# sundy-li/strawboat

Measured on AMD Instinct MI355X. Metric: encode+decode GB/s (uncompressed Arrow bytes) per GPU; 1/2/4/8-GPU scaling, higher is better.
Workload: dtype f64 bit patterns (integer/bit work, no arithmetic); 1 GPU; C2: 512 x 1M-row nullable Float64 columns per GPU, 64Ki-row pages, codec adaptive, inputs resident in HBM; columns_per_gpu=512, rows_per_column=1000000, page_rows=65536, parallelism=pages of independent columns sharded across 1 GPU(s)

## Files before the change

### strawboat_amd/csrc/sb_encode.hip

```cpp
#include <cstring>
#include <type_traits>
#include <utility>
#include <vector>

#include "sb_host.h"
#include "sb_lz4.h"
#include "sb_zstd_enc.h"

namespace sb {

struct EncCol {
    const uint8_t* values;
    const uint8_t* validity;
    const uint8_t* offsets;
    const uint8_t* heads;
    uint8_t* out;
    uint64_t values_bit_offset;
    uint64_t values_len;
    uint64_t values_len_total;
    uint64_t validity_bit_offset;
    uint64_t out_cap;
    uint64_t rows;
    int32_t ptype;
    int32_t nullable;
// ... 3056 lines not shown
#include "sb_select_big.h"
#include "sb_dict_big.h"
#include "sb_bin_page.h"

constexpr uint32_t BIN_LDS_SLOTS = 16384;

constexpr uint32_t BH_ROWS = 2048;
#ifndef BV_ROWS_
#define BV_ROWS_ 4096
#endif
constexpr uint32_t BV_ROWS = BV_ROWS_;
__global__ void __launch_bounds__(WG) k_enc_bin_hash(EncodeArgs a) {
    const uint32_t page = blockIdx.x + a.page_base;
    const EncPage p = get_page(a, page);
    if (p.codec != CODEC_ON_DEVICE || p.h64_off == ~0ull) return;
    const uint64_t r0 = (uint64_t)blockIdx.y * BH_ROWS;
    if (r0 >= p.rows) return;
    if (bp_page_done(a, p, page)) return;
    const EncCol c = get_col(a, p.col);
    const uint64_t r1 = min(p.rows, r0 + BH_ROWS);
    uint64_t* h64 = (uint64_t*)(a.scratch + p.h64_off);
    auto body = [&](auto bk) {
        constexpr int U = 8;
        for (uint64_t base = r0 + threadIdx.x; base < r1; base += (uint64_t)WG * U) {
            uint64_t b[U], e[U];
#pragma unroll
            for (int u = 0; u < U; u++) {
                const uint64_t i = base + (uint64_t)u * WG;
                const uint64_t ic = i < r1 ? i : r0;
                b[u] = bk.beg(ic);
                e[u] = bk.beg(ic + 1);
            }
#pragma unroll
            for (int u = 0; u < U; u++) {
                const uint64_t i = base + (uint64_t)u * WG;
                if (i < r1) gst64(h64 + i, bin_hash_bytes(bk.values, b[u], e[u], c.values_len));
            }
        }
    };
    const ValidView vv{c.validity, c.validity_bit_offset + p.row0};
    if (c.ptype == SB_TYPE_BINARY)
        body(BinKeys<int32_t>{c.offsets + p.row0 * 4, c.values, vv});
    else if (c.ptype == SB_TYPE_LARGE_BINARY)
        body(BinKeys<int64_t>{c.offsets + p.row0 * 8, c.values, vv});
}

__global__ void __launch_bounds__(WG) k_enc_bin_verify(EncodeArgs a, uint32_t tiles_per_page) {
    const uint32_t lin = blockIdx.x, xcd = lin & 7, j = lin >> 3;
    const uint32_t pidx = (j / tiles_per_page) * 8 + xcd, tile = j % tiles_per_page;
    if (pidx >= a.n_pages) return;
    const uint32_t page = pidx + a.page_base;
    const EncPage p = get_page(a, page);
    if (p.codec != CODEC_ON_DEVICE || p.h64_off == ~0ull || !p.aux_bytes) return;
    const uint64_t r0 = (uint64_t)tile * BV_ROWS;
    if (r0 >= p.rows) return;
    if (bp_page_done(a, p, page)) return;
    uint32_t* aux = (uint32_t*)(a.scratch + p.aux_off);
    if (!bh_fits(p.rows, p.aux_bytes)) return;
    const uint32_t magic = gld32(aux + BH_W_MAGIC);
    if (magic != BH_MAGIC && magic != BH_TAGS_USED) return;
    if (a.flags & SB_WRITE_DEBUG_VERIFY_FAIL_BIT) {
        if (threadIdx.x == 0 && tile == 0) atomicOr(aux + BH_W_BAD, 1u);
        return;
    }
    const EncCol c = get_col(a, p.col);
    const uint64_t r1 = min(p.rows, r0 + BV_ROWS);
    const ValidView vv{c.validity, c.validity_bit_offset + p.row0};
    const uint16_t* slot16 = (const uint16_t*)(aux + BH_W_SLOT16);
    const uint16_t* rep16 = (const uint16_t*)(aux + BH_W_REP16);
    const uint64_t* h64 = (const uint64_t*)(a.scratch + p.h64_off);
    bool ok = true;
    auto body = [&](auto keys) {
        using KT = decltype(keys);
        constexpr int VU = 8;
        constexpr bool O32 = sizeof(keys.k.beg(0)) == 8 && std::is_same<KT, BinKeysHashed<int32_t>>::value;
        const uint8_t* offs = keys.k.offs;
        const uint8_t* values = keys.k.values;
        const uint64_t vlen = c.values_len;
        for (uint64_t base = r0 + threadIdx.x; base < r1; base += (uint64_t)WG * VU) {
            uint32_t g[VU];
            uint64_t br[VU], er[VU], bg[VU], eg[VU];
            bool need[VU];
#pragma unroll
            for (int u = 0; u < VU; u++) {
                const uint64_t row = base + (uint64_t)u * WG;
                const uint64_t rc = row < r1 ? row : r0;
                g[u] = ldu16((const uint8_t*)(rep16 + ldu16((const uint8_t*)(slot16 + rc))));
                need[u] = row < r1 && g[u] != (uint32_t)rc;
                if (!need[u]) g[u] = (uint32_t)rc;
            }
#pragma unroll
            for (int u = 0; u < VU; u++) {
                const uint64_t row = base + (uint64_t)u * WG;
                const uint64_t rc = row < r1 ? row : r0;
                if constexpr (O32) {
                    const uint64_t pr = ldu64(offs + rc * 4), pg = ldu64(offs + (uint64_t)g[u] * 4);
                    br[u] = (uint32_t)pr; er[u] = pr >> 32; bg[u] = (uint32_t)pg; eg[u] = pg >> 32;
                } else {
                    br[u] = keys.k.beg(rc); er[u] = keys.k.beg(rc + 1); bg[u] = keys.k.beg(g[u]); eg[u] = keys.k.beg((uint64_t)g[u] + 1);
                }
            }
#pragma unroll
            for (int u = 0; u < VU; u++) {
                if (!need[u]) continue;
                const uint64_t n = er[u] - br[u];
                if (n != eg[u] - bg[u]) {
                    ok = false;
                    continue;
                }
                if (n <= 32 && br[u] + 32 <= vlen && bg[u] + 32 <= vlen) {
                    const u32x4 a4 = ldu128(values + br[u]), b4 = ldu128(values + bg[u]);
                    const u32x4 a5 = ldu128(values + br[u] + 16), b5 = ldu128(values + bg[u] + 16);
                    auto msk = [](uint64_t have) -> uint64_t { return have >= 8 ? ~0ull : ((1ull << (8 * have)) - 1); };
                    const uint64_t d0 = ((uint64_t)(a4.x ^ b4.x)) | ((uint64_t)(a4.y ^ b4.y) << 32), d1 = ((uint64_t)(a4.z ^ b4.z)) | ((uint64_t)(a4.w ^ b4.w) << 32);
                    const uint64_t d2 = ((uint64_t)(a5.x ^ b5.x)) | ((uint64_t)(a5.y ^ b5.y) << 32), d3 = ((uint64_t)(a5.z ^ b5.z)) | ((uint64_t)(a5.w ^ b5.w) << 32);
                    const uint64_t x = (d0 & msk(n)) | (d1 & msk(n > 8 ? n - 8 : 0)) | (d2 & msk(n > 16 ? n - 16 : 0)) | (d3 & msk(n > 24 ? n - 24 : 0));
                    if (x) ok = false;
                } else {
                    const uint64_t row = base + (uint64_t)u * WG;
                    if (!keys.k.eq(g[u], row)) ok = false;
                }
            }
        }
    };
    if (c.ptype == SB_TYPE_BINARY)
        body(BinKeysHashed<int32_t>{BinKeys<int32_t>{c.offsets + p.row0 * 4, c.values, vv}, h64, c.values_len});
    else
        body(BinKeysHashed<int64_t>{BinKeys<int64_t>{c.offsets + p.row0 * 8, c.values, vv}, h64, c.values_len});
    if (!ok) atomicOr(aux + BH_W_BAD, 1u);
}

template <int KIND>
__global__ void __launch_bounds__(WG) k_enc_select(EncodeArgs a) {
    constexpr uint32_t LDS_SLOTS = KIND < 0 ? BIN_LDS_SLOTS : SEL_LDS_SLOTS;
    __shared__ uint32_t lds_tab[LDS_SLOTS];
    __shared__ uint32_t s_misc[2 * WG + 16];
    constexpr int SMP = SAMPLE_CAP * ((KIND > 0 ? KIND : 1) + 1) + 16, STR = 1024 + 4 * 96 * (KIND == 8 ? 8 : 4) + 4 * 96;
    __shared__ __attribute__((aligned(16))) uint8_t sample_mem[SMP > STR ? SMP : STR];
    static_assert(KIND >= 0 || LDS_SLOTS >= BH_SLOTS + 4096, "tag slots + the hand-over's bitmap and prefix share lds_tab");
    __shared__ uint32_t s_tagged;
    const uint32_t page = spread_block(blockIdx.x, gridDim.x) + a.page_base;
    const EncPage p = get_page(a, page);
    if (p.codec != CODEC_ON_DEVICE) return;
    const EncCol c = get_col(a, p.col);
    if (c.ptype == SB_TYPE_NULL) return;
    const bool is_bool = c.ptype == SB_TYPE_BOOLEAN;
    const bool is_bin = c.ptype == SB_TYPE_BINARY || c.ptype == SB_TYPE_LARGE_BINARY;
    if constexpr (KIND == 0) {
        if (!is_bool) return;
    } else if constexpr (KIND == -4) {
        if (c.ptype != SB_TYPE_BINARY) return;
    } else if constexpr (KIND == -8) {
        if (c.ptype != SB_TYPE_LARGE_BINARY) return;
    } else {
        if (is_bool || is_bin || c.width != (uint32_t)KIND) return;
    }
    const uint64_t N = p.rows;
    if constexpr (KIND == 1 || KIND == 2) {
        if (a.use_counts && !a.redo && a.page_base == 0 && page < a.n_pages && N >= SEL_BIG_ROWS) {
            if (threadIdx.x == 0) a.codecs[page] = CODEC_PENDING;
            return;
        }
    }
    if constexpr (KIND < 0) {
        if (bp_page_done(a, p, page)) return;
        if (a.use_counts && !a.redo && a.page_base == 0 && page < a.n_pages && N >= BIN_BIG_ROWS && p.bigx_off && p.h64_off != ~0ull &&
            a.pre_hashed) {
            if (threadIdx.x == 0) a.codecs[page] = CODEC_PENDING;
            return;
        }
    }
    const ValidView vv{c.validity, c.validity_bit_offset + p.row0};
    SelectOpts so{a.ratio, a.has_ratio, a.forbidden | p.forb_extra, a.default_compression, -1, p.seed, p.depth};
    SelScratch sc{lds_tab, s_misc, sample_mem, p.aux_bytes ? (uint32_t*)(a.scratch + p.aux_off) : nullptr, 0};
    sc.lds_slots = LDS_SLOTS;
    if (sc.gtab) {
        uint64_t M = 64;
        while (M < 2 * N) M <<= 1;
        sc.gslots = M;
    }
    uint32_t codec;
    bool handover = false;
    if constexpr (KIND < 0) {
        if (threadIdx.x == 0) s_tagged = 0;
        const bool fits = p.h64_off != ~0ull && page < a.n_pages && sc.gtab && bh_fits(N, p.aux_bytes) && !((a.forbidden >> SB_CODEC_DICT) & 1);
        if (a.redo) {
            if (!fits) return;
            const uint32_t magic = gld32(sc.gtab + BH_W_MAGIC);
            if ((magic != BH_MAGIC && magic != BH_TAGS_USED) || gld32(sc.gtab + BH_W_BAD) == 0) return;
            if (threadIdx.x == 0) {
                const uint32_t old = (uint32_t)a.codecs[page];
                atomicSub(&a.codec_counts[old & 31], 1u);
                if (old == SB_CODEC_FREQ) atomicSub(a.freq_count, 1u);
            }
        } else if (fits) {
            handover = true;
            sc.slot16 = (uint16_t*)(sc.gtab + BH_W_SLOT16);
            sc.tagged = &s_tagged;
        }
        __syncthreads();
        if (threadIdx.x == 0 && sc.gtab && p.aux_bytes >= 64) {
            gst32(sc.gtab + BH_W_MAGIC, 0u);
            gst32(sc.gtab + BH_W_BAD, 0u);
        }
        __syncthreads();
    } else {
        if (a.redo) return;
    }
    if constexpr (KIND == 0) {
        codec = choose_bool(c.values, c.values_bit_offset + p.row0, vv, N, so, sc);
    } else if constexpr (KIND == -4) {
        BinKeys<int32_t> bk{c.offsets + p.row0 * 4, c.values, vv};
        codec = choose_bin<int32_t>(bk, N, c.values_len_total, so, sc, p.h64_off != ~0ull ? (uint64_t*)(a.scratch + p.h64_off) : nullptr, c.values_len,
                                    a.pre_hashed != 0);
        __syncthreads();
        if (handover && s_tagged) {
            if (codec == SB_CODEC_DICT)
                bin_dict_handover<int32_t>(bk, N, lds_tab, lds_tab + BH_SLOTS, s_misc, sc.gtab);
            else if (threadIdx.x == 0)
                gst32(sc.gtab + BH_W_MAGIC, BH_TAGS_USED);
        }
        STL(46);
    } else if constexpr (KIND == -8) {
        BinKeys<int64_t> bk{c.offsets + p.row0 * 8, c.values, vv};
        codec = choose_bin<int64_t>(bk, N, c.values_len_total, so, sc, p.h64_off != ~0ull ? (uint64_t*)(a.scratch + p.h64_off) : nullptr, c.values_len,
                                    a.pre_hashed != 0);
        __syncthreads();
        if (handover && s_tagged) {
            if (codec == SB_CODEC_DICT)
                bin_dict_handover<int64_t>(bk, N, lds_tab, lds_tab + BH_SLOTS, s_misc, sc.gtab);
            else if (threadIdx.x == 0)
                gst32(sc.gtab + BH_W_MAGIC, BH_TAGS_USED);
        }
    } else {
        const uint8_t* vals = c.values + p.row0 * KIND;
        codec = choose_prim<KIND>([=](uint64_t i) { return ld_val<KIND>(vals + i * KIND); }, vv, N, c.nk, so, sc);
    }
    if (threadIdx.x == 0) {
        a.codecs[page] = (int32_t)codec;
        atomicAdd(&a.codec_counts[codec & 31], 1u);
        if (!has_device_encoder(codec))
            raise(a.status, SB_ERR_NYI, page, 700 + codec);
        else if (codec == SB_CODEC_FREQ && page < a.n_pages)
            atomicAdd(a.freq_count, 1u);
    }
}

template <int KIND, int FK>
__global__ void __launch_bounds__(WG, 4) k_enc_select_rle(EncodeArgs a) {
    __shared__ uint32_t lds_tab[SEL_LDS_SLOTS];
    __shared__ uint32_t s_misc[2 * WG + 16];
    __shared__ __attribute__((aligned(16))) uint8_t sample_mem[SAMPLE_CAP * (KIND + 1) + 16];
    __shared__ uint32_t s_cnt2[2];
    if (a.codec_counts[HINT_ROW_SELECT] == 0) return;
    const uint32_t page = blockIdx.x;
    const EncPage p = a.pages[page];
    if (p.codec != CODEC_ON_DEVICE) return;
    const EncCol c = a.cols[p.col];
    if (c.ptype == SB_TYPE_NULL || c.ptype == SB_TYPE_BOOLEAN || c.ptype == SB_TYPE_BINARY || c.ptype == SB_TYPE_LARGE_BINARY) return;
    if (c.width != (uint32_t)KIND || (c.fkind != 0) != (FK != 0)) return;
    if (a.codecs[page] != CODEC_PENDING) return;
    const uint64_t N = p.rows;
    if (N >= SEL_BIG_ROWS) return;
    SelectOpts so{a.ratio, a.has_ratio, a.forbidden | p.forb_extra, a.default_compression, -1, p.seed, p.depth};
    SelScratch sc{lds_tab, s_misc, sample_mem, p.aux_bytes ? (uint32_t*)(a.scratch + p.aux_off) : nullptr, 0};
    if (sc.gtab) {
        uint64_t M = 64;
        while (M < 2 * N) M <<= 1;
        sc.gslots = M;
    }
    uint32_t codec = so.default_codec;
    bool kept = false;
    if (N > 0) codec = select_rle_page<KIND, FK>(a, c, p, page, so, sc, s_cnt2, &kept);
    if (threadIdx.x == 0) {
        a.codecs[page] = (int32_t)codec;
        if (!kept) atomicAdd(&a.codec_counts[codec & 31], 1u);
        if (!has_device_encoder(codec))
            raise(a.status, SB_ERR_NYI, page, 700 + codec);
        else if (codec == SB_CODEC_FREQ)
            atomicAdd(a.freq_count, 1u);
    }
}

#ifndef SB_RUNS_OCC
#define SB_RUNS_OCC 4
#endif
template <int KIND, int FK>
__global__ void __launch_bounds__(WG, SB_RUNS_OCC) k_enc_select_runs(EncodeArgs a) {
    __shared__ uint32_t lds_tab[SEL_LDS_SLOTS];
    constexpr int SMP_BYTES = (SAMPLE_CAP * (KIND + 1) + 16 + 15) / 16 * 16, MISC_BYTES = (2 * WG + 16) * 4;
    __shared__ __attribute__((aligned(16))) uint8_t pool[SMP_BYTES + MISC_BYTES];
    uint8_t* sample_mem = pool;
    uint32_t* s_misc = (uint32_t*)(pool + SMP_BYTES);
    __shared__ uint32_t s_cnt2[2];
    static_assert(SMP_BYTES + MISC_BYTES >= 2 * (RUNS_CAP + 8) + (WG * 16 / 32 + 32) * 4 + 8 * KIND + (RUNS_CAP + 1) * KIND,
                  "run list and run values must fit the pool");
    const uint32_t page = blockIdx.x;
    const EncPage p = a.pages[page];
    if (p.codec != CODEC_ON_DEVICE) return;
    const EncCol c = a.cols[p.col];
    if (c.ptype == SB_TYPE_NULL || c.ptype == SB_TYPE_BOOLEAN || c.ptype == SB_TYPE_BINARY || c.ptype == SB_TYPE_LARGE_BINARY) return;
    if (c.width != (uint32_t)KIND || (c.fkind != 0) != (FK != 0)) return;
    const uint64_t N = p.rows;
    if (N >= SEL_BIG_ROWS) {
        if (threadIdx.x == 0) {
            a.codecs[page] = CODEC_PENDING;
            atomicAdd(&a.codec_counts[HINT_ROW_SELECT], 1u);
        }
        return;
    }
    SelectOpts so{a.ratio, a.has_ratio, a.forbidden | p.forb_extra, a.default_compression, -1, p.seed, p.depth};
    SelScratch sc{lds_tab, s_misc, sample_mem, p.aux_bytes ? (uint32_t*)(a.scratch + p.aux_off) : nullptr, 0};
    if (sc.gtab) {
        uint64_t M = 64;
        while (M < 2 * N) M <<= 1;
        sc.gslots = M;
    }
    uint32_t codec = so.default_codec;
    bool kept = false, fallback = false;
    if (N > 0) codec = select_runs_page<KIND, FK>(a, c, p, page, so, sc, s_cnt2, &kept, &fallback);
    if (threadIdx.x == 0) {
        if (fallback) {
            a.codecs[page] = CODEC_PENDING;
            atomicAdd(&a.codec_counts[HINT_ROW_SELECT], 1u);
            return;
        }
        a.codecs[page] = (int32_t)codec;
        if (!kept) atomicAdd(&a.codec_counts[codec & 31], 1u);
        if (!has_device_encoder(codec))
            raise(a.status, SB_ERR_NYI, page, 700 + codec);
        else if (codec == SB_CODEC_FREQ)
            atomicAdd(a.freq_count, 1u);
    }
}

typedef void (*EncSelectKernel)(EncodeArgs);
static EncSelectKernel enc_select_kernel(int kind) {
    switch (kind) {
        case 0:
            return k_enc_select<0>;
        case 1:
            return k_enc_select<1>;
        case 2:
            return k_enc_select<2>;
        case 4:
            return k_enc_select<4>;
        case 8:
            return k_enc_select<8>;
        case 16:
            return k_enc_select<16>;
        case 32:
            return k_enc_select<32>;
        case -4:
            return k_enc_select<-4>;
        case -8:
            return k_enc_select<-8>;
    }
    return nullptr;
}

template <int KIND, int CODEC>
constexpr int emit_pages_occupancy() {
    return CODEC == SB_CODEC_DICT ? 2 : CODEC == SB_CODEC_PATAS ? 1 : ((CODEC == SB_CODEC_ONEVALUE || CODEC == SB_CODEC_RLE) && KIND == 32) ? 3
           : (CODEC == SB_CODEC_RLE || CODEC == SB_CODEC_ONEVALUE) ? 4 : 3;
}
template <int KIND, int CODEC>
__global__ void __launch_bounds__(WG, (emit_pages_occupancy<KIND, CODEC>()))
    k_enc_emit_pages(EncodeArgs a) {
    constexpr int LW = CODEC == SB_CODEC_ONEVALUE ? 256
                       : CODEC == SB_CODEC_RLE ? (int)(RleRows<(KIND > 0 ? KIND : 1)>::WORDS + 2) / 3
                                               : SIDX_WORDS;
    constexpr uint32_t BIN_TABLE = (KIND < 0 && CODEC == SB_CODEC_DICT) ? BIN_LDS_SLOTS : 1;
    constexpr int LDS_MIN = (KIND < 0 && CODEC == SB_CODEC_DICT) ? 2 * LW + (int)BH_SLOTS / 2 : 0;
    constexpr int LDS_WORDS0 = 3 * LW > (int)BIN_TABLE ? 3 * LW : (int)BIN_TABLE;
    constexpr int LDS_WORDS = LDS_WORDS0 > LDS_MIN ? LDS_WORDS0 : LDS_MIN;
    __shared__ __attribute__((aligned(16))) uint32_t lds[LDS_WORDS];
    uint32_t *sA = lds, *sB = lds + LW, *sC = lds + 2 * LW;
    uint32_t* const s_bin_table = lds;
    __shared__ uint32_t s_w[4];
    if (a.use_counts && a.codec_counts[CODEC] == 0) return;
    const uint32_t page = spread_block(blockIdx.x, gridDim.x) + a.page_base;
    const EncPage p = get_page(a, page);
    if (codec_of(a, p, page) != CODEC) return;
    if constexpr (CODEC == SB_CODEC_RLE || CODEC == SB_CODEC_DICT) {
        if (a.outs[page].pad == 1 && a.outs[page].length != 0) return;
    }
    if constexpr (CODEC == SB_CODEC_DICT) {
        if ((a.skips & SKIP_DICT_BIG) && p.bigx_off && page < a.n_pages) return;
    }
    const EncCol c = get_col(a, p.col);
    if (c.ptype == SB_TYPE_NULL) return;
    const bool is_bool = c.ptype == SB_TYPE_BOOLEAN;
    const bool is_bin = c.ptype == SB_TYPE_BINARY || c.ptype == SB_TYPE_LARGE_BINARY;
    if constexpr (KIND == 0) {
        if (!is_bool) return;
    } else if constexpr (KIND == -4) {
        if (c.ptype != SB_TYPE_BINARY) return;
    } else if constexpr (KIND == -8) {
        if (c.ptype != SB_TYPE_LARGE_BINARY) return;
    } else {
        if (is_bool || is_bin || c.width != (uint32_t)KIND) return;
    }
    if constexpr (CODEC == SB_CODEC_RLE && (KIND == 4 || KIND == 8)) {
        if (threadIdx.x == 0 && a.use_counts) atomicAdd(&a.codec_counts[HINT_RLE_EMIT], 1u);
    }
    if constexpr (CODEC == SB_CODEC_DICT && KIND < 0) {
        if (threadIdx.x == 0 && a.use_counts) atomicAdd(&a.codec_counts[HINT_BIN_DICT_EMIT], 1u);
    }
    uint8_t* slot = page_slot(a, c, p);
    const uint64_t N = p.rows;
    uint64_t pos = 0;
    ValidView vv{c.validity, c.validity_bit_offset + p.row0};
    if (c.nullable) {
        uint8_t* bits = def_header(slot, N);
        def_bits_page(bits, ValidView{c.validity, c.validity_bit_offset}, p.row0, N, c.rows);
        pos = def_section_bytes(N);
    }
    uint64_t blen = 0;
    uint8_t* blk = slot + pos;
    if constexpr (KIND == 0)
        blen = emit_bool_page<CODEC>(a, c, p, page, blk, vv, sA, sB, sC, s_w);
    else if constexpr (KIND == -4)
        blen = emit_binary_page<int32_t, CODEC>(a, c, p, page, blk, vv, sA, sB, sC, s_w, s_bin_table, BIN_TABLE);
    else if constexpr (KIND == -8)
        blen = emit_binary_page<int64_t, CODEC>(a, c, p, page, blk, vv, sA, sB, sC, s_w, s_bin_table, BIN_TABLE);
    else
        blen = emit_prim_page<KIND, CODEC>(a, c, p, page, blk, vv, sA, sB, sC, s_w);
    if (threadIdx.x == 0) {
        EncOut o;
        o.length = blen == DICT_FREQ_PENDING ? 1 : (blen ? pos + blen : 0);
        o.out_off = 0;
        o.slot = slot;
        o.codec = (uint32_t)CODEC;
        o.pad = blen == DICT_FREQ_PENDING ? 3 : 0;
        a.outs[page] = o;
    }
}

typedef void (*EncPageKernel)(EncodeArgs);
template <int KIND>
static EncPageKernel enc_page_kernel_for_codec(int32_t codec) {
    switch (codec) {
        case SB_CODEC_RLE:
            return k_enc_emit_pages<KIND, SB_CODEC_RLE>;
        case SB_CODEC_DICT:
            return k_enc_emit_pages<KIND, SB_CODEC_DICT>;
        case SB_CODEC_ONEVALUE:
            return k_enc_emit_pages<KIND, SB_CODEC_ONEVALUE>;
        case SB_CODEC_BITPACKING:
            return k_enc_emit_pages<KIND, SB_CODEC_BITPACKING>;
        case SB_CODEC_DELTA_BITPACKING:
            return k_enc_emit_pages<KIND, SB_CODEC_DELTA_BITPACKING>;
        case SB_CODEC_PATAS:
            if constexpr (KIND == 4 || KIND == 8) return k_enc_emit_pages<KIND, SB_CODEC_PATAS>;
            return nullptr;
    }
    return nullptr;
}
static EncPageKernel enc_page_kernel(int kind, int32_t codec) {
    switch (kind) {
        case 0:
            return enc_page_kernel_for_codec<0>(codec);
        case 1:
            return enc_page_kernel_for_codec<1>(codec);
        case 2:
            return enc_page_kernel_for_codec<2>(codec);
        case 4:
            return enc_page_kernel_for_codec<4>(codec);
        case 8:
            return enc_page_kernel_for_codec<8>(codec);
        case 16:
            return enc_page_kernel_for_codec<16>(codec);
        case 32:
            return enc_page_kernel_for_codec<32>(codec);
        case -4:
            return enc_page_kernel_for_codec<-4>(codec);
        case -8:
            return enc_page_kernel_for_codec<-8>(codec);
    }
    return nullptr;
}

__device__ uint32_t zstd_store_frame_wg(const uint8_t* src, uint32_t n, uint8_t* dst, uint32_t* s4) {
    if (threadIdx.x == 0) {
        stu32(dst, 0xFD2FB528u);
        dst[4] = (uint8_t)((3u << 6) | (1u << 5));
        stu64(dst + 5, (uint64_t)n);
    }
    uint32_t op = 13, pos = 0;
    do {
        const uint32_t len = min(128u * 1024u, n - pos);
        const bool last = pos + len == n;
        uint32_t diff = 0;
        for (uint32_t i = threadIdx.x; i < len; i += WG) diff |= src[pos + i] != src[pos];
        const bool rle = len > 0 && wg_or32(diff, s4) == 0;
        if (threadIdx.x == 0) {
            const uint32_t hdr = (last ? 1u : 0u) | ((rle ? 1u : 0u) << 1) | (len << 3);
            dst[op] = (uint8_t)hdr;
            dst[op + 1] = (uint8_t)(hdr >> 8);
            dst[op + 2] = (uint8_t)(hdr >> 16);
            if (rle) dst[op + 3] = src[pos];
        }
        op += 3;
        if (rle) {
            op += 1;
        } else {
            wg_copy(dst + op, src + pos, len);
            op += len;
        }
        pos += len;
    } while (pos < n);
    __syncthreads();
    return op;
}

constexpr uint32_t FREQ_MAX_CONTAINERS = 1024;
template <class IsExc, class OnExc>
__device__ void freq_roaring(uint64_t N, uint8_t* rb, uint8_t* size_field, uint32_t* sA, uint32_t* s_w, uint32_t* s_card,
                             IsExc is_exc, OnExc on_exc, uint32_t& rb_size_out, uint32_t& n_ex_out) {
    const int t = threadIdx.x, lane = t & 63;
    const uint32_t nc_all = (uint32_t)((N + 65535) / 65536);
    for (uint32_t q = t; q < FREQ_MAX_CONTAINERS; q += WG) s_card[q] = 0;
    __syncthreads();
    for (uint32_t cq = 0; cq < nc_all; cq++) {
        const uint64_t b = (uint64_t)cq * 65536, e = min(N, b + 65536);
        uint32_t cnt = 0;
        for (uint64_t i = b + t; i < e; i += WG) cnt += is_exc(i) ? 1u : 0u;
        const uint32_t tot = wg_sum32(cnt, s_w);
        if (t == 0) s_card[cq] = tot;
    }
    __syncthreads();
    uint32_t ncne = 0, n_ex = 0;
    for (uint32_t cq = 0; cq < nc_all; cq++) {
        ncne += s_card[cq] ? 1u : 0u;
        n_ex += s_card[cq];
    }
    uint32_t rb_size = 8 + 8 * ncne;
    for (uint32_t cq = 0; cq < nc_all; cq++)
        if (s_card[cq]) rb_size += s_card[cq] > 4096 ? 8192u : 2 * s_card[cq];
    if (t == 0) {
        stu32(size_field, rb_size);
        stu32(rb, 12346u);
        stu32(rb + 4, ncne);
        uint32_t k = 0, off = 8 + 8 * ncne;
        for (uint32_t cq = 0; cq < nc_all; cq++) {
            if (!s_card[cq]) continue;
            *(gptr)(rb + 8 + 4 * k) = (uint8_t)cq;
            *(gptr)(rb + 8 + 4 * k + 1) = (uint8_t)(cq >> 8);
            *(gptr)(rb + 8 + 4 * k + 2) = (uint8_t)(s_card[cq] - 1);
            *(gptr)(rb + 8 + 4 * k + 3) = (uint8_t)((s_card[cq] - 1) >> 8);
            stu32(rb + 8 + 4 * ncne + 4 * k, off);
            off += s_card[cq] > 4096 ? 8192u : 2 * s_card[cq];
            k++;
        }
    }
    uint32_t data_off = 8 + 8 * ncne, ex_base = 0;
    for (uint32_t cq = 0; cq < nc_all; cq++) {
        const uint32_t card = s_card[cq];
        if (!card) continue;
        const bool bitmap = card > 4096;
        const uint64_t b = (uint64_t)cq * 65536, e = min(N, b + 65536);
        if (bitmap)
            for (uint32_t i = t; i < 2048; i += WG) stu32(rb + data_off + 4 * i, 0);
        __syncthreads();
        uint32_t carry = 0;
        for (uint64_t cb = b; cb < e; cb += TILE_ROWS) {
            const uint32_t n = (uint32_t)min((uint64_t)TILE_ROWS, e - cb);
            bool f[ROWS_PER_THREAD];
#pragma unroll
            for (int j = 0; j < ROWS_PER_THREAD; j++) {
                const uint32_t r = (uint32_t)t + (uint32_t)j * WG;
                f[j] = r < n && is_exc(cb + r);
                sA[sidx((int)r)] = f[j] ? 1u : 0u;
                if (bitmap) {
                    const uint64_t m = __ballot(f[j]);
                    if (lane == 0 && (r & ~63u) < n) stu64(rb + data_off + ((cb - b + (r & ~63u)) >> 6) * 8, m);
                }
            }
            __syncthreads();
            const uint32_t tot = tile_incl_scan(sA, s_w);
#pragma unroll
            for (int j = 0; j < ROWS_PER_THREAD; j++) {
                const uint32_t r = (uint32_t)t + (uint32_t)j * WG;
                if (!f[j]) continue;
                const uint32_t k = carry + sA[sidx((int)r)] - 1;
                if (!bitmap) {
                    const uint32_t lo16 = (uint32_t)(cb - b) + r;
                    *(gptr)(rb + data_off + 2 * k) = (uint8_t)lo16;
                    *(gptr)(rb + data_off + 2 * k + 1) = (uint8_t)(lo16 >> 8);
                }
                on_exc(cb + r, ex_base + k);
            }
            carry += tot;
            __syncthreads();
        }
        data_off += bitmap ? 8192u : 2 * card;
        ex_base += card;
    }
    rb_size_out = rb_size;
    n_ex_out = n_ex;
}

template <int W>
struct FreqKeys {
    const uint8_t* vals;
    uint32_t nk;
// ... 2228 lines not shown
```

### strawboat_amd/csrc/sb_select_runs.h

```cpp
#ifndef SB_RUNS_LANE_ROWS
#define SB_RUNS_LANE_ROWS 1
#endif
constexpr int32_t CODEC_PENDING = -100;
constexpr uint32_t RUNS_CAP = 640;

#if SB_RUNS_LANE_ROWS
template <int W>
__device__ __forceinline__ Val<W> wave_shr1_val(const Val<W>& v, const Val<W>& lane0) {
    int a[W / 4], o[W / 4], b[W / 4];
    __builtin_memcpy(a, &v, W);
    __builtin_memcpy(o, &lane0, W);
#pragma unroll
    for (int k = 0; k < W / 4; k++) b[k] = __builtin_amdgcn_update_dpp(o[k], a[k], 0x138 , 0xF, 0xF, false);
    Val<W> r;
    __builtin_memcpy(&r, b, W);
    return r;
}
#endif

template <int W, int FK>
__device__ uint32_t select_runs_page(const EncodeArgs& a, const EncCol& c, const EncPage& p, uint32_t page, const SelectOpts& o,
                                     const SelScratch& sc, uint32_t* s_cnt2 , bool* rle_kept, bool* fallback) {
    static_assert(W == 4 || W == 8, "fused select + RLE: 4- and 8-byte values");
    constexpr int K = 16;
    constexpr uint32_t CHUNK = WG * K;
    constexpr int REC = 4 + W;
    constexpr uint64_t SENT = ~0ull;
    constexpr uint32_t KSLOTS = SEL_LDS_SLOTS / 2, KCAP = KSLOTS / 2;
    const int t = threadIdx.x, lane = t & 63;
    const int w = __builtin_amdgcn_readfirstlane((int)(threadIdx.x >> 6));
    const uint64_t lt = (1ull << lane) - 1;
    const uint64_t N = p.rows;
    const uint8_t* vals = c.values + p.row0 * W;
    const ValidView vv{c.validity, c.validity_bit_offset + p.row0};
    const uint32_t nk = c.nk;
    const bool is_float = nk >= NK_F32;
    auto getv = [=](uint64_t i) { return ld_val<W>(vals + i * W); };
    auto forbidden = [&](uint32_t cd) { return (o.forbidden >> cd) & 1u; };
    auto k64 = [&](const Val<W>& k) {
        uint64_t x = 0;
        __builtin_memcpy(&x, &k, W);
        return x;
    };
    *rle_kept = false;
    *fallback = false;
    const Val<W> k0 = stat_key<W>(getv(0), nk);
    uint32_t f_neq0 = 0, f_unsorted = 0, f_neg = 0, nulls = 0;
    Val<W> tmax = getv(0);
    uint64_t vote_k = 0;
    uint32_t vote_n = 0;
    unsigned long long* kset = (unsigned long long*)sc.lds_tab;
    uint32_t& s_kcnt = s_cnt2[0];
    uint32_t& s_ksent = s_cnt2[1];
    const bool want_set = !forbidden(SB_CODEC_DICT) && N >= 3;
    const bool want_vote = !forbidden(SB_CODEC_FREQ);
    for (uint32_t i = t; i < KSLOTS; i += WG) kset[i] = SENT;
    if (t == 0) {
        s_kcnt = 0;
        s_ksent = 0;
    }
    uint16_t* runs = (uint16_t*)sc.sample_mem;
    uint32_t* s_vb = (uint32_t*)(sc.sample_mem + 2 * (RUNS_CAP + 8));
    uint32_t* s_x = s_vb + CHUNK / 32;
    Val<W>* s_lastk = (Val<W>*)(s_x + 32);
    Val<W>* rvals = s_lastk + 8;
    __syncthreads();
    bool spec = !forbidden(SB_CODEC_RLE);
    uint8_t* slot = page_slot(a, c, p);
    const uint64_t pos = c.nullable ? def_section_bytes(N) : 0;
    uint8_t* dst = slot + pos + 9;
    uint64_t run_start = 0;
    uint32_t nrec = 0;
    bool have = false;
    Val<W> last = val_zero<W>();
    const uint64_t vtotal = vv.off + N;
    auto lds_barrier = []() {
        __builtin_amdgcn_fence(__ATOMIC_RELEASE, "workgroup", "local");
        __builtin_amdgcn_s_barrier();
        __builtin_amdgcn_fence(__ATOMIC_ACQUIRE, "workgroup", "local");
    };
    uint32_t par = 0;
    Val<W> v[K];
    Val<W> pv0 = val_zero<W>();
    uint32_t vword = 0;
#if SB_RUNS_LANE_ROWS
    constexpr int PR = 16 / W, NP = K / PR;
    const uint32_t wrow = (uint32_t)w * (64 * K), lrow = wrow + (uint32_t)lane * PR;
    auto request = [&](uint64_t cb) {
        const uint32_t n = (uint32_t)min((uint64_t)CHUNK, N - cb);
        if (wrow + 64 * K <= n) {
#pragma unroll
            for (int u = 0; u < NP; u++) {
                const u32x4 q = ldu128(vals + (cb + lrow + (uint32_t)u * 64 * PR) * W);
                __builtin_memcpy(&v[u * PR], &q, 16);
            }
        } else {
#pragma unroll
            for (int u = 0; u < NP; u++) {
                const uint32_t r = lrow + (uint32_t)u * 64 * PR;
                if (r + PR <= n) {
                    const u32x4 q = ldu128(vals + (cb + r) * W);
                    __builtin_memcpy(&v[u * PR], &q, 16);
                } else {
#pragma unroll
                    for (int i = 0; i < PR; i++) v[u * PR + i] = getv(cb + (r + i < n ? r + i : n - 1));
                }
            }
        }
        if (lane == 0) pv0 = getv(cb + wrow > 0 ? min(cb + wrow - 1, N - 1) : 0);
        vword = 0xFFFFFFFFu;
        if (t < (int)(CHUNK / 32) && (uint32_t)t * 32 < n && vv.bits) vword = bits32(vv.bits, vv.off + cb + (uint32_t)t * 32, vtotal);
    };
#else
    auto request = [&](uint64_t cb) {
        const uint32_t n = (uint32_t)min((uint64_t)CHUNK, N - cb);
        const uint32_t r0 = (uint32_t)t * K;
        if (r0 + K <= n) {
            constexpr int NV = K * W / 16;
            u32x4 q[NV];
#pragma unroll
            for (int u = 0; u < NV; u++) q[u] = ldu128(vals + (cb + r0) * W + 16 * u);
            __builtin_memcpy(v, q, K * W);
        } else {
#pragma unroll
            for (int j = 0; j < K; j++) v[j] = getv(cb + (r0 + j < n ? r0 + j : n - 1));
        }
        if (lane == 0) pv0 = getv(cb + r0 > 0 ? min(cb + r0 - 1, N - 1) : 0);
        vword = 0xFFFFFFFFu;
        if (t < (int)(CHUNK / 32) && (uint32_t)t * 32 < n && vv.bits) vword = bits32(vv.bits, vv.off + cb + (uint32_t)t * 32, vtotal);
    };
#endif
    STL(0);
    for (uint64_t cb = 0; cb < N; cb += CHUNK) {
        XTL(0);
        request(cb);
        const uint32_t n = (uint32_t)min((uint64_t)CHUNK, N - cb);
        if (t < (int)(CHUNK / 32)) {
            const uint32_t b0 = (uint32_t)t * 32;
            uint32_t word = 0;
            if (b0 < n) {
                const uint32_t nb = min(32u, n - b0);
                const uint32_t m = nb >= 32 ? 0xFFFFFFFFu : (1u << nb) - 1;
                word = vword & m;
                nulls += nb - (uint32_t)__popc(word);
            }
            s_vb[t] = word;
        }
        uint32_t* s_rc = s_x + par * 16 + 12;
#if SB_RUNS_LANE_ROWS
        if (t == 0) rvals[0] = pv0;
        bool chg[K];
        uint32_t cnt_p[NP];
        uint32_t cnt_w = 0;
        {
            Val<W> carry = readlane_val<W>(pv0, 0);
#pragma unroll
            for (int u = 0; u < NP; u++) {
                uint32_t c = 0;
#pragma unroll
                for (int i = 0; i < PR; i++) {
                    const Val<W> pr = i ? v[u * PR + i - 1] : wave_shr1_val<W>(v[u * PR + PR - 1], carry);
                    bool ne = !bits_eq<W>(v[u * PR + i], pr);
                    if (u == 0 && i == 0) ne = ne || t == 0;
                    ne = ne && lrow + (uint32_t)(u * 64 * PR + i) < n;
                    chg[u * PR + i] = ne;
                    c += (uint32_t)__popcll(__ballot(ne));
                }
                cnt_p[u] = c;
                cnt_w += c;
                carry = readlane_val<W>(v[u * PR + PR - 1], 63);
            }
        }
        XTL(1);
        if (lane == 0) s_rc[w] = cnt_w;
#else
        const uint32_t r0 = (uint32_t)t * K;
        const uint32_t mine = r0 < n ? min((uint32_t)K, n - r0) : 0u;
        Val<W> pvrow = shfl_val<W>(v[K - 1], (lane + 63) & 63);
        if (lane == 0) pvrow = pv0;
        if (t == 0) rvals[0] = pvrow;
        uint32_t rbm = 0;
        {
            Val<W> pr = pvrow;
#pragma unroll
            for (int j = 0; j < K; j++) {
                if (!bits_eq<W>(v[j], pr)) rbm |= 1u << j;
                pr = v[j];
            }
            if (r0 == 0) rbm |= 1u;
            rbm &= mine >= (uint32_t)K ? 0xFFFFu : ((1u << mine) - 1);
        }
        XTL(1);
        const uint32_t cnt1 = (uint32_t)__popc(rbm);
        const uint32_t incl1 = wave_incl_scan(cnt1);
        if (lane == 63) s_rc[w] = incl1;
#endif
        lds_barrier();
        XTL(2);
        const uint32_t total = s_rc[0] + s_rc[1] + s_rc[2] + s_rc[3];
        if (total > RUNS_CAP) {
            *fallback = true;
            return 0;
        }
#if SB_RUNS_LANE_ROWS
        {
            uint32_t base = 0;
            for (int pw = 0; pw < 3; pw++)
                if (pw < w) base += s_rc[pw];
#pragma unroll
            for (int u = 0; u < NP; u++) {
                uint32_t at = base;
#pragma unroll
                for (int i = 0; i < PR; i++) at += mbcnt64(__ballot(chg[u * PR + i]));
#pragma unroll
                for (int i = 0; i < PR; i++) {
                    if (chg[u * PR + i]) {
                        runs[at] = (uint16_t)(lrow + (uint32_t)(u * 64 * PR + i));
                        rvals[1 + at] = v[u * PR + i];
                    }
                    at += chg[u * PR + i];
                }
                base += cnt_p[u];
            }
            if (t == 0) runs[total] = (uint16_t)n;
        }
#else
        {
            uint32_t at = incl1 - cnt1;
            for (int pw = 0; pw < 3; pw++)
                if (pw < w) at += s_rc[pw];
            while (rbm) {
                const int j = __ffs((int)rbm) - 1;
                rbm &= rbm - 1;
                Val<W> x = v[0];
#pragma unroll
                for (int q = 1; q < K; q++)
                    if (j == q) x = v[q];
                runs[at] = (uint16_t)(r0 + (uint32_t)j);
                rvals[1 + at] = x;
                at++;
            }
            if (t == 0) runs[total] = (uint16_t)n;
        }
#endif
        XTL(3);
        lds_barrier();
        XTL(4);
        for (uint32_t rb = 0; rb < total; rb += WG, par ^= 1) {
            const uint32_t r = rb + (uint32_t)t;
            const bool act = r < total;
            const uint32_t start = act ? runs[r] : 0, end = act ? runs[r + 1] : 0;
            const uint64_t row = cb + start;
            const Val<W> val = rvals[act ? 1 + r : 0];
            const Val<W> kk = stat_key<W>(val, nk);
            if (act) {
                if (!bits_eq<W>(kk, k0)) f_neq0 = 1;
                if (!is_float) {
                    if (int_lt<W>(tmax, val, nk)) tmax = val;
                    if (W == 4 && nk == NK_SIGNED && (int32_t)as_i64<W>(val, nk) < 0) f_neg = 1;
                    if (W == 4 && row > 0 && int_lt<W>(val, rvals[r], nk)) f_unsorted = 1;
                }
                if (want_vote) {
                    const uint64_t x = k64(kk);
                    const uint32_t wgt = end - start;
                    if (vote_k == x) {
                        vote_n += wgt;
                    } else if (vote_n >= wgt) {
                        vote_n -= wgt;
                    } else {
                        vote_k = x;
                        vote_n = wgt - vote_n;
                    }
                }
                if (want_set && s_kcnt <= KCAP) {
                    const uint64_t x = k64(kk);
                    if (x == SENT) {
                        s_ksent = 1;
                    } else {
                        uint32_t h = (((uint32_t)x ^ (uint32_t)(x >> 32) * 0x85EBCA6Bu) * 0x9E3779B1u >> 15) & (KSLOTS - 1);
                        for (;;) {
                            unsigned long long cur = kset[h];
                            if (cur == x) break;
                            if (cur == SENT) {
                                const unsigned long long old = atomicCAS(&kset[h], (unsigned long long)SENT, (unsigned long long)x);
                                if (old == SENT) {
                                    atomicAdd(&s_kcnt, 1u);
                                    break;
                                }
                                if (old == x) break;
                            }
                            h = (h + 1) & (KSLOTS - 1);
                        }
                    }
                }
            }
            XTL(5);
            if (!spec) continue;
            int fv = -1;
            if (act) {
                const uint32_t w0 = start >> 5, w1 = (end - 1) >> 5;
                for (uint32_t wd = w0; wd <= w1; wd++) {
                    uint32_t bits = s_vb[wd];
                    if (wd == w0) bits &= 0xFFFFFFFFu << (start & 31);
                    if (wd == w1 && (end & 31)) bits &= (1u << (end & 31)) - 1;
                    if (bits) {
                        fv = (int)(wd * 32) + __ffs((int)bits) - 1;
                        break;
                    }
                }
            }
            const bool hv = fv >= 0;
            uint32_t* s_has = s_x + par * 16;
            uint32_t* s_cnt = s_x + par * 16 + 4;
            uint32_t* s_blast = s_x + par * 16 + 8;
            Val<W>* s_last = s_lastk + par * 4;
            const uint64_t hm = __ballot(hv);
            const bool has_w = hm != 0;
            const Val<W> last_w = readlane_val<W>(kk, has_w ? top_bit(hm) : 0);
            if (lane == 0) {
                s_has[w] = has_w;
                s_last[w] = last_w;
            }
            XTL(6);
            lds_barrier();
            XTL(7);
            bool chas = have;
            Val<W> cval = last;
            for (int pw = 0; pw < 3; pw++)
                if (pw < w && s_has[pw]) {
                    chas = true;
                    cval = s_last[pw];
                }
            const uint64_t pm = hm & lt;
            const Val<W> pvs = shfl_val<W>(kk, pm ? top_bit(pm) : 0);
            const bool pc = pm ? true : chas;
            const Val<W> pvk = pm ? pvs : cval;
            if (hv && !pc) st_val<W>(dst + 4, val);
            const bool b = hv && pc && !bits_eq<W>(pvk, kk);
            const uint64_t bmk = __ballot(b);
            const uint32_t blast = b ? (uint32_t)fv + 1 : 0;
            const uint64_t pb = bmk & lt;
            const uint32_t prev_blast = __shfl(blast, pb ? top_bit(pb) : 0, 64);
            const uint32_t cnt_w = (uint32_t)__popcll(bmk);
            const uint32_t blast_w = (uint32_t)__builtin_amdgcn_readlane((int)blast, bmk ? top_bit(bmk) : 0);
            if (lane == 0) {
                s_cnt[w] = cnt_w;
                s_blast[w] = bmk ? blast_w : 0;
            }
            XTL(8);
            lds_barrier();
            XTL(9);
            uint32_t base = nrec;
            uint64_t start_prev = run_start;
            for (int pw = 0; pw < 3; pw++)
                if (pw < w) {
                    base += s_cnt[pw];
                    if (s_blast[pw]) start_prev = cb + s_blast[pw] - 1;
                }
            if (b) {
                uint8_t* rec = dst + (uint64_t)(base + (uint32_t)__popcll(pb)) * REC;
                const uint64_t sr = pb ? cb + prev_blast - 1 : start_prev;
                stu32(rec, (uint32_t)(cb + (uint32_t)fv - sr));
                st_val<W>(rec + REC + 4, val);
            }
            for (int pw = 0; pw < 4; pw++) {
                if (s_has[pw]) {
                    have = true;
                    last = s_last[pw];
                }
                nrec += s_cnt[pw];
                if (s_blast[pw]) run_start = cb + s_blast[pw] - 1;
            }
        }
        XTL(10);
        if (!spec) lds_barrier();
        if ((uint64_t)nrec * 4 > cb + n + 256) spec = false;
    }
    __syncthreads();
    STL(1);
    PrimPartials<W> pp{f_neq0, f_unsorted, f_neg, nulls, tmax, vote_k, vote_n};
    const uint32_t s_k = want_set ? s_kcnt : 0u, s_s = want_set ? s_ksent : 0u;
    SamplePre<W> none;
    __builtin_memset(&none, 0, sizeof none);
    const uint32_t codec = decide_prim<W>(getv, vv, N, nk, o, sc, pp, want_set, want_vote, s_k, s_s, none, none, none, none, false);
    if (codec == SB_CODEC_RLE && spec) {
        if (t == 0) {
            uint8_t* r = dst + (uint64_t)nrec * REC;
            stu32(r, (uint32_t)(N - run_start));
            if (!have) st_val<W>(r + 4, val_zero<W>());
        }
        if (c.nullable) {
            uint8_t* bits = def_header(slot, N);
            def_bits_page(bits, ValidView{c.validity, c.validity_bit_offset}, p.row0, N, c.rows);
        }
        const uint64_t body = (uint64_t)(nrec + 1) * REC;
        if (t == 0) {
            put_hdr9(slot + pos, SB_CODEC_RLE, (uint32_t)body, (uint32_t)(N * W));
            EncOut out;
            out.length = pos + 9 + body;
            out.out_off = 0;
            out.slot = slot;
            out.codec = SB_CODEC_RLE;
            out.pad = 1;
            a.outs[page] = out;
        }
        *rle_kept = true;
    }
    return codec;
}
```

Baseline: 3789 GB/s.

## Specialize run-selector chunks for full tiles and use 32-bit page indexing

After: 3758 GB/s. Within noise of the previous version (-0.8%).

```diff
diff --git a/strawboat_amd/csrc/sb_encode.hip b/strawboat_amd/csrc/sb_encode.hip
--- a/strawboat_amd/csrc/sb_encode.hip
+++ b/strawboat_amd/csrc/sb_encode.hip
@@ -3382,6 +3382,7 @@
     if (c.ptype == SB_TYPE_NULL || c.ptype == SB_TYPE_BOOLEAN || c.ptype == SB_TYPE_BINARY || c.ptype == SB_TYPE_LARGE_BINARY) return;
     if (c.width != (uint32_t)KIND || (c.fkind != 0) != (FK != 0)) return;
     const uint64_t N = p.rows;
+    static_assert(SEL_BIG_ROWS * 16 <= 1ull << 32, "pages of the run-level selector: 32-bit rows and byte offsets");
     if (N >= SEL_BIG_ROWS) {
         if (threadIdx.x == 0) {
             a.codecs[page] = CODEC_PENDING;
diff --git a/strawboat_amd/csrc/sb_select_runs.h b/strawboat_amd/csrc/sb_select_runs.h
--- a/strawboat_amd/csrc/sb_select_runs.h
+++ b/strawboat_amd/csrc/sb_select_runs.h
@@ -17,6 +17,26 @@
     return r;
 }
 #endif
+
+template <bool B>
+struct BoolC {
+    static constexpr bool value = B;
+};
+
+template <bool LONG>
+__device__ __forceinline__ uint32_t bits32_page(const uint8_t* p, uint32_t pos, uint32_t nbytes) {
+    const uint32_t b0 = pos >> 3, sh = pos & 7;
+    uint64_t v = 0;
+    if (LONG || nbytes >= 8) {
+        const uint32_t b = b0 + 8 <= nbytes ? b0 : nbytes - 8;
+        v = ldu64(p + b);
+        const uint32_t skip = (b0 - b) * 8;
+        v = skip < 64 ? v >> skip : 0;
+    } else {
+        for (uint32_t k = 0; k < 8 && b0 + k < nbytes; k++) v |= (uint64_t)ldu8(p + b0 + k) << (8 * k);
+    }
+    return (uint32_t)(v >> sh);
+}
 
 template <int W, int FK>
 __device__ uint32_t select_runs_page(const EncodeArgs& a, const EncCol& c, const EncPage& p, uint32_t page, const SelectOpts& o,
@@ -30,12 +50,15 @@
     const int t = threadIdx.x, lane = t & 63;
     const int w = __builtin_amdgcn_readfirstlane((int)(threadIdx.x >> 6));
     const uint64_t lt = (1ull << lane) - 1;
-    const uint64_t N = p.rows;
+    const uint32_t N = (uint32_t)p.rows;
     const uint8_t* vals = c.values + p.row0 * W;
     const ValidView vv{c.validity, c.validity_bit_offset + p.row0};
+    const uint8_t* vbits = vv.bits ? vv.bits + (vv.off >> 3) : nullptr;
+    const uint32_t voff = (uint32_t)(vv.off & 7), vbytes = (voff + N + 7) >> 3;
     const uint32_t nk = c.nk;
     const bool is_float = nk >= NK_F32;
     auto getv = [=](uint64_t i) { return ld_val<W>(vals + i * W); };
+    auto getv32 = [=](uint32_t i) { return ld_val<W>(vals + i * W); };
     auto forbidden = [&](uint32_t cd) { return (o.forbidden >> cd) & 1u; };
     auto k64 = [&](const Val<W>& k) {
         uint64_t x = 0;
@@ -69,11 +92,10 @@
     uint8_t* slot = page_slot(a, c, p);
     const uint64_t pos = c.nullable ? def_section_bytes(N) : 0;
     uint8_t* dst = slot + pos + 9;
-    uint64_t run_start = 0;
+    uint32_t run_start = 0;
     uint32_t nrec = 0;
     bool have = false;
     Val<W> last = val_zero<W>();
-    const uint64_t vtotal = vv.off + N;
     auto lds_barrier = []() {
         __builtin_amdgcn_fence(__ATOMIC_RELEASE, "workgroup", "local");
         __builtin_amdgcn_s_barrier();
@@ -86,12 +108,15 @@
 #if SB_RUNS_LANE_ROWS
     constexpr int PR = 16 / W, NP = K / PR;
     const uint32_t wrow = (uint32_t)w * (64 * K), lrow = wrow + (uint32_t)lane * PR;
-    auto request = [&](uint64_t cb) {
-        const uint32_t n = (uint32_t)min((uint64_t)CHUNK, N - cb);
-        if (wrow + 64 * K <= n) {
+#endif
+    auto chunk_runs = [&](auto full_c, const uint32_t cb, const uint32_t n) -> uint32_t {
+        constexpr bool FULL = decltype(full_c)::value;
+        const uint8_t* cvals = vals + cb * W;
+#if SB_RUNS_LANE_ROWS
+        if (FULL || wrow + 64 * K <= n) {
 #pragma unroll
             for (int u = 0; u < NP; u++) {
-                const u32x4 q = ldu128(vals + (cb + lrow + (uint32_t)u * 64 * PR) * W);
+                const u32x4 q = ldu128(cvals + lrow * W + u * (64 * 16));
                 __builtin_memcpy(&v[u * PR], &q, 16);
             }
         } else {
@@ -99,82 +124,67 @@
             for (int u = 0; u < NP; u++) {
                 const uint32_t r = lrow + (uint32_t)u * 64 * PR;
                 if (r + PR <= n) {
-                    const u32x4 q = ldu128(vals + (cb + r) * W);
+                    const u32x4 q = ldu128(cvals + r * W);
                     __builtin_memcpy(&v[u * PR], &q, 16);
                 } else {
 #pragma unroll
-                    for (int i = 0; i < PR; i++) v[u * PR + i] = getv(cb + (r + i < n ? r + i : n - 1));
-                }
-            }
-        }
-        if (lane == 0) pv0 = getv(cb + wrow > 0 ? min(cb + wrow - 1, N - 1) : 0);
-        vword = 0xFFFFFFFFu;
-        if (t < (int)(CHUNK / 32) && (uint32_t)t * 32 < n && vv.bits) vword = bits32(vv.bits, vv.off + cb + (uint32_t)t * 32, vtotal);
-    };
+                    for (int i = 0; i < PR; i++) v[u * PR + i] = ld_val<W>(cvals + (r + i < n ? r + i : n - 1) * W);
+                }
+            }
+        }
+        const uint32_t r0 = wrow;
 #else
-    auto request = [&](uint64_t cb) {
-        const uint32_t n = (uint32_t)min((uint64_t)CHUNK, N - cb);
         const uint32_t r0 = (uint32_t)t * K;
         if (r0 + K <= n) {
             constexpr int NV = K * W / 16;
             u32x4 q[NV];
 #pragma unroll
-            for (int u = 0; u < NV; u++) q[u] = ldu128(vals + (cb + r0) * W + 16 * u);
+            for (int u = 0; u < NV; u++) q[u] = ldu128(cvals + r0 * W + 16 * u);
             __builtin_memcpy(v, q, K * W);
         } else {
 #pragma unroll
-            for (int j = 0; j < K; j++) v[j] = getv(cb + (r0 + j < n ? r0 + j : n - 1));
-        }
-        if (lane == 0) pv0 = getv(cb + r0 > 0 ? min(cb + r0 - 1, N - 1) : 0);
+            for (int j = 0; j < K; j++) v[j] = ld_val<W>(cvals + (r0 + j < n ? r0 + j : n - 1) * W);
+        }
+#endif
+        if (lane == 0) pv0 = getv32(cb + r0 > 0 ? (FULL ? cb + r0 - 1 : min(cb + r0 - 1, N - 1)) : 0);
         vword = 0xFFFFFFFFu;
-        if (t < (int)(CHUNK / 32) && (uint32_t)t * 32 < n && vv.bits) vword = bits32(vv.bits, vv.off + cb + (uint32_t)t * 32, vtotal);
-    };
-#endif
-    STL(0);
-    for (uint64_t cb = 0; cb < N; cb += CHUNK) {
-        XTL(0);
-        request(cb);
-        const uint32_t n = (uint32_t)min((uint64_t)CHUNK, N - cb);
+        if (t < (int)(CHUNK / 32) && (FULL || (uint32_t)t * 32 < n) && vbits) vword = bits32_page<FULL>(vbits, voff + cb + (uint32_t)t * 32, vbytes);
         if (t < (int)(CHUNK / 32)) {
-            const uint32_t b0 = (uint32_t)t * 32;
-            uint32_t word = 0;
-            if (b0 < n) {
-                const uint32_t nb = min(32u, n - b0);
-                const uint32_t m = nb >= 32 ? 0xFFFFFFFFu : (1u << nb) - 1;
-                word = vword & m;
+            uint32_t word = vword;
+            if (!FULL) {
+                const uint32_t b0 = (uint32_t)t * 32;
+                const uint32_t nb = b0 < n ? min(32u, n - b0) : 0u;
+                word &= nb >= 32 ? 0xFFFFFFFFu : (1u << nb) - 1;
                 nulls += nb - (uint32_t)__popc(word);
+            } else {
+                nulls += 32 - (uint32_t)__popc(word);
             }
             s_vb[t] = word;
         }
         uint32_t* s_rc = s_x + par * 16 + 12;
 #if SB_RUNS_LANE_ROWS
-        if (t == 0) rvals[0] = pv0;
-        bool chg[K];
-        uint32_t cnt_p[NP];
+        if (w == 0 && lane == 0) rvals[0] = pv0;
+        uint64_t chg[K];
         uint32_t cnt_w = 0;
         {
             Val<W> carry = readlane_val<W>(pv0, 0);
 #pragma unroll
             for (int u = 0; u < NP; u++) {
-                uint32_t c = 0;
 #pragma unroll
                 for (int i = 0; i < PR; i++) {
                     const Val<W> pr = i ? v[u * PR + i - 1] : wave_shr1_val<W>(v[u * PR + PR - 1], carry);
-                    bool ne = !bits_eq<W>(v[u * PR + i], pr);
-                    if (u == 0 && i == 0) ne = ne || t == 0;
-                    ne = ne && lrow + (uint32_t)(u * 64 * PR + i) < n;
-                    chg[u * PR + i] = ne;
-                    c += (uint32_t)__popcll(__ballot(ne));
-                }
-                cnt_p[u] = c;
-                cnt_w += c;
+                    uint64_t m = __ballot(!bits_eq<W>(v[u * PR + i], pr));
+                    if (!FULL) m &= __ballot(lrow + (uint32_t)(u * 64 * PR + i) < n);
+                    if (u == 0 && i == 0) m |= (uint64_t)(w == 0);
+                    chg[u * PR + i] = m;
+                    cnt_w += (uint32_t)__popcll(m);
+                }
                 carry = readlane_val<W>(v[u * PR + PR - 1], 63);
             }
         }
         XTL(1);
         if (lane == 0) s_rc[w] = cnt_w;
 #else
-        const uint32_t r0 = (uint32_t)t * K;
         const uint32_t mine = r0 < n ? min((uint32_t)K, n - r0) : 0u;
         Val<W> pvrow = shfl_val<W>(v[K - 1], (lane + 63) & 63);
         if (lane == 0) pvrow = pv0;
@@ -197,32 +207,40 @@
 #endif
         lds_barrier();
         XTL(2);
-        const uint32_t total = s_rc[0] + s_rc[1] + s_rc[2] + s_rc[3];
+        uint32_t rc[4];
+#pragma unroll
+        for (int pw = 0; pw < 4; pw++) rc[pw] = (uint32_t)__builtin_amdgcn_readfirstlane((int)s_rc[pw]);
+        const uint32_t total = rc[0] + rc[1] + rc[2] + rc[3];
         if (total > RUNS_CAP) {
             *fallback = true;
-            return 0;
+            return ~0u;
         }
 #if SB_RUNS_LANE_ROWS
         {
             uint32_t base = 0;
             for (int pw = 0; pw < 3; pw++)
-                if (pw < w) base += s_rc[pw];
+                if (pw < w) base += rc[pw];
 #pragma unroll
             for (int u = 0; u < NP; u++) {
                 uint32_t at = base;
 #pragma unroll
-                for (int i = 0; i < PR; i++) at += mbcnt64(__ballot(chg[u * PR + i]));
-#pragma unroll
                 for (int i = 0; i < PR; i++) {
-                    if (chg[u * PR + i]) {
-                        runs[at] = (uint16_t)(lrow + (uint32_t)(u * 64 * PR + i));
-                        rvals[1 + at] = v[u * PR + i];
+                    const uint64_t m = chg[u * PR + i];
+                    at = __builtin_amdgcn_mbcnt_hi((uint32_t)(m >> 32), __builtin_amdgcn_mbcnt_lo((uint32_t)m, at));
+                    base += (uint32_t)__popcll(m);
+                }
+#pragma unroll
+                for (int i = 0; i < PR; i++) {
+                    const bool own = __builtin_amdgcn_inverse_ballot_w64(chg[u * PR + i]);
+                    if (own) {
+                        const uint32_t at2 = at * 2;
+                        *(uint16_t*)((uint8_t*)runs + at2) = (uint16_t)(lrow + (uint32_t)(u * 64 * PR + i));
+                        *(Val<W>*)((uint8_t*)(rvals + 1) + at2 * (W / 2)) = v[u * PR + i];
                     }
-                    at += chg[u * PR + i];
-                }
-                base += cnt_p[u];
-            }
-            if (t == 0) runs[total] = (uint16_t)n;
+                    if (i + 1 < PR) at += own;
+                }
+            }
+            if (w == 0 && lane == 0) runs[total] = (uint16_t)n;
         }
 #else
         {
@@ -246,12 +264,21 @@
         XTL(3);
         lds_barrier();
         XTL(4);
+        return total;
+    };
+    STL(0);
+    for (uint32_t cb = 0; cb < N; cb += CHUNK) {
+        XTL(0);
+        const uint32_t n = min(CHUNK, N - cb);
+        const uint32_t total = n == CHUNK ? chunk_runs(BoolC<true>{}, cb, CHUNK) : chunk_runs(BoolC<false>{}, cb, n);
+        if (total == ~0u) return 0;
         for (uint32_t rb = 0; rb < total; rb += WG, par ^= 1) {
             const uint32_t r = rb + (uint32_t)t;
             const bool act = r < total;
-            const uint32_t start = act ? runs[r] : 0, end = act ? runs[r + 1] : 0;
-            const uint64_t row = cb + start;
-            const Val<W> val = rvals[act ? 1 + r : 0];
+            const uint32_t rr = min(r, RUNS_CAP - 1);
+            const uint32_t start = runs[rr], end = runs[rr + 1];
+            const uint32_t row = cb + start;
+            const Val<W> val = rvals[1 + rr];
             const Val<W> kk = stat_key<W>(val, nk);
             if (act) {
                 if (!bits_eq<W>(kk, k0)) f_neq0 = 1;
@@ -351,16 +378,16 @@
             lds_barrier();
             XTL(9);
             uint32_t base = nrec;
-            uint64_t start_prev = run_start;
+            uint32_t start_prev = run_start;
             for (int pw = 0; pw < 3; pw++)
                 if (pw < w) {
                     base += s_cnt[pw];
                     if (s_blast[pw]) start_prev = cb + s_blast[pw] - 1;
                 }
             if (b) {
-                uint8_t* rec = dst + (uint64_t)(base + (uint32_t)__popcll(pb)) * REC;
-                const uint64_t sr = pb ? cb + prev_blast - 1 : start_prev;
-                stu32(rec, (uint32_t)(cb + (uint32_t)fv - sr));
+                uint8_t* rec = dst + (base + (uint32_t)__popcll(pb)) * REC;
+                const uint32_t sr = pb ? cb + prev_blast - 1 : start_prev;
+                stu32(rec, cb + (uint32_t)fv - sr);
                 st_val<W>(rec + REC + 4, val);
             }
             for (int pw = 0; pw < 4; pw++) {
```
